# Bebra777228/PolGen-RVC

Measured on AMD Instinct MI355X. Metric: real-time-factor (audio-sec/wall-sec) per GPU, 30s@16kHz RMVPE->48kHz, higher is better.
Workload: dtype f32 (conv products as 3 fp16 MFMAs of a hi/lo split, fp32 accumulate; fp32 elsewhere)

## Files before the change

include/rvcx.h:

```cpp
#ifndef RVCX_H
#define RVCX_H
#include <stdint.h>

#ifdef __cplusplus
extern "C" {
#endif

typedef struct rvcx_ctx rvcx_ctx;

typedef struct {
  const char* name;
  const void* data;
  int32_t dtype;
  int32_t ndim;
  int64_t shape[4];
} rvcx_tensor;

typedef struct {
  int32_t inter_channels, hidden_channels, filter_channels, n_heads, n_layers, kernel_size;
  int32_t n_resblocks;
  int32_t res_kernels[4];
  int32_t res_dilations[4][3];
  int32_t n_ups;
  int32_t up_rates[6], up_kernels[6];
// ... 253 lines not shown
                   int pad_left, int Tout, int groups, int pre_lrelu, float pre_slope, int act,
                   float act_slope, const int32_t* lens_in, const int32_t* lens_out);
int rvcx_op_resblock_pair(rvcx_ctx*, const float* x, const float* w1, const float* b1, const float* w2,
                          const float* b2, float* y, int B, int C, int T, int K, int dil, float slope, int fused,
                          const int32_t* lens);
int rvcx_op_resblock3(rvcx_ctx*, const float* x, const float* w1, const float* b1, const float* w2, const float* b2,
                      float* y, int B, int C, int T, const int32_t* dils, float slope, const int32_t* lens);
int rvcx_bench_resblock_pair(rvcx_ctx*, int B, int C, int T, int K, int dil, int fused, int iters,
                             float* ms_per_launch);
int rvcx_bench_conv1d(rvcx_ctx*, int B, int Cin, int Tin, int Cout, int K, int stride, int dil, int groups,
                      int iters, float* ms_per_launch);
int rvcx_conv_override(int tile, int variant, int splitk);
int rvcx_op_convtranspose1d(rvcx_ctx*, const float* x, const float* w, const float* bias, float* y,
                            int B, int Cin, int Tin, int Cout, int K, int stride, int pad,
                            int pre_lrelu, float pre_slope);
int rvcx_op_conv2d3x3(rvcx_ctx*, const float* x, const float* w, const float* bias, const float* res,
                      float* y, int B, int Cin, int H, int W, int Cout, int act);
int rvcx_op_convblock2d(rvcx_ctx*, const float* x, const float* w1, const float* b1, const float* w2, const float* b2,
                        const float* wsc, const float* bsc, float* y, int B, int Cin, int Cout, int H, int W,
                        const int32_t* rows);
int rvcx_op_convtranspose2d(rvcx_ctx*, const float* x, const float* w, const float* bias, float* y,
                            int B, int Cin, int H, int W, int Cout, int act);
int rvcx_op_attention(rvcx_ctx*, const float* q, const float* k, const float* v, float* out, int B,
                      int H, int D, int T, float scale, const float* emb_rel_k,
                      const float* emb_rel_v, int window, const int32_t* lens);
int rvcx_op_gemm_tm(rvcx_ctx*, const float* x_cf, const float* w, const float* bias, const float* res_tm, int B, int T,
                    int Cin, int Cout, int act, int exact_fp32, float* y_tm, float* y_cf, float* y_split);
int rvcx_bench_gemm(rvcx_ctx*, int64_t rows, int Cin, int Cout, int iters, float* ms_per_launch);
int rvcx_op_layernorm_tm(rvcx_ctx*, const float* x, const float* gamma, const float* beta, float* y, float* y_split,
                         int64_t rows, int C, float eps);
// ... 35 lines not shown
```

polgen-rvc_amd/_lib.py:

```python
from __future__ import annotations

import ctypes as C
import os
import threading
import types
from typing import Optional, Sequence

import numpy as np

_HERE = os.path.dirname(os.path.abspath(__file__))
LIB_PATH = os.environ.get("RVCX_LIBRARY") or os.path.join(_HERE, "librvcx.so")


class RvcxError(RuntimeError):
    pass


class Tensor(C.Structure):
    _fields_ = [("name", C.c_char_p), ("data", C.c_void_p), ("dtype", C.c_int32),
                ("ndim", C.c_int32), ("shape", C.c_int64 * 4)]


class SynthCfg(C.Structure):
    _fields_ = [("inter_channels", C.c_int32), ("hidden_channels", C.c_int32),
# ... 98 lines not shown
    k = min(Lx, Lb)
    fin = np.sin(0.5 * np.pi * np.arange(Lx) / max(Lx - 1, 1)) ** 2
    out[:k] = y[d:d + k] * fin[:k] + b[:k] * (1.0 - fin[:k])
    return out, y[d + Lb:d + Lb + Lx].copy(), d, scores, mags


_lib = None

SYMBOLS = [
    "rvcx_create", "rvcx_destroy", "rvcx_last_error", "rvcx_version", "rvcx_load_hubert",
    "rvcx_load_rmvpe", "rvcx_index_exhaustive", "rvcx_load_crepe", "rvcx_crepe_frames", "rvcx_crepe_predict", "rvcx_op_crepe_decode", "rvcx_get_f0_crepe_x", "rvcx_load_fcpe", "rvcx_fcpe_f0", "rvcx_fcpe_frames", "rvcx_get_f0_fcpe_x", "rvcx_op_fcpe_post", "rvcx_load_synth", "rvcx_unload_synth", "rvcx_load_index", "rvcx_load_index_ivf",
    "rvcx_weights_regions", "rvcx_weights_adopt", "rvcx_weights_clone", "rvcx_rmvpe_f0", "rvcx_rmvpe_frames", "rvcx_rmvpe_mel", "rvcx_synth_infer_taps", "rvcx_hubert_features",
    "rvcx_hubert_frames", "rvcx_synth_infer", "rvcx_synth_infer_window", "rvcx_synth_dec_rf", "rvcx_synth_upp", "rvcx_index_blend",
    "rvcx_out_len", "rvcx_convert_batch", "rvcx_convert_batch_f64", "rvcx_micro_batch", "rvcx_bucket_length", "rvcx_last_micro_batches", "rvcx_last_cuts", "rvcx_noise_len",
    "rvcx_get_f0", "rvcx_get_f0_x", "rvcx_vc", "rvcx_vc_frames", "rvcx_last_timing",
    "rvcx_flop_counter", "rvcx_fp32_reruns", "rvcx_mem_info", "rvcx_conv_profile", "rvcx_conv_profile_csv", "rvcx_stream", "rvcx_op_conv1d", "rvcx_op_resblock_pair", "rvcx_bench_resblock_pair", "rvcx_bench_conv1d", "rvcx_conv_override", "rvcx_op_convtranspose1d",
    "rvcx_op_conv2d3x3", "rvcx_op_convblock2d", "rvcx_op_convtranspose2d", "rvcx_op_attention", "rvcx_op_layernorm_c",
    "rvcx_op_bigru", "rvcx_op_highpass", "rvcx_highpass_exact", "rvcx_convert_batch_ex", "rvcx_get_f0_x_ex", "rvcx_fp32_layers", "rvcx_fp32_pinned",
    "rvcx_gru_fallbacks", "rvcx_gru_publish_probe", "rvcx_debug_inject", "rvcx_f0_file_track", "rvcx_op_gemm_tm", "rvcx_op_layernorm_tm",
    "rvcx_resample_len", "rvcx_resample_f64", "rvcx_resample_f64_kind", "rvcx_bench_gemm", "rvcx_device_info",
    "rvcx_convert_submit", "rvcx_convert_wait", "rvcx_convert_poll", "rvcx_convert_inflight", "rvcx_ticket_lead_ms",
    "rvcx_synth_infer_head", "rvcx_op_sola", "rvcx_stream_open", "rvcx_stream_step", "rvcx_stream_reset", "rvcx_stream_close",
    "rvcx_stream_out_len", "rvcx_stream_noise_len", "rvcx_stream_frames",
    "rvcx_stream_open_io", "rvcx_stream_in_len", "rvcx_stream_delays", "rvcx_stream_resample_delay", "rvcx_stream_last_taps",
    "rvcx_stream_set", "rvcx_op_stream_resample",
    "rvcx_stream_open_fx", "rvcx_stream_out_channels", "rvcx_stream_set_fx", "rvcx_stream_last_fx_ms", "rvcx_op_stream_fx",
    "rvcx_fx_reverb_host",
    "rvcx_fx_chain", "rvcx_op_fx_highpass", "rvcx_op_fx_compressor", "rvcx_op_fx_gate", "rvcx_op_fx_reverb", "rvcx_op_fx_shelf",
    "rvcx_op_fx_chorus", "rvcx_op_fx_mix", "rvcx_fx_chunk", "rvcx_fx_last_passes", "rvcx_fx_cte", "rvcx_fx_delay",
    "rvcx_fx_coeffs", "rvcx_fx_highpass_host", "rvcx_fx_biquad_host", "rvcx_fx_follower_host", "rvcx_fx_compressor_host",
    "rvcx_fx_gate_host", "rvcx_fx_comb_host", "rvcx_fx_allpass_host", "rvcx_fx_chorus_host", "rvcx_fx_mix_host",
# ... 568 lines not shown
        return ms.value, flops / (ms.value * 1e-3) / 1e12

    def convtranspose1d(self, x, w, bias=None, stride=1, pad=0, pre_lrelu=None):
        x, w = f32(x), f32(w)
        B, Cin, Tin = x.shape
        _, Cout, K = w.shape
        Tout = (Tin - 1) * stride - 2 * pad + K
        y = np.empty((B, Cout, Tout), np.float32)
        bias = None if bias is None else f32(bias)
        self._ck(lib().rvcx_op_convtranspose1d(self._h, _p(x), _p(w), _p(bias), _p(y), B, Cin, Tin, Cout, K,
                                               stride, pad, 0 if pre_lrelu is None else 1,
                                               C.c_float(0.0 if pre_lrelu is None else pre_lrelu)),
                 "op_convtranspose1d")
        return y

    def conv2d3x3(self, x, w, bias=None, res=None, act=0):
        x, w = f32(x), f32(w)
        B, Cin, H, W = x.shape
        Cout = w.shape[0]
        y = np.empty((B, Cout, H, W), np.float32)
        bias = None if bias is None else f32(bias)
        res = None if res is None else f32(res)
        self._ck(lib().rvcx_op_conv2d3x3(self._h, _p(x), _p(w), _p(bias), _p(res), _p(y), B, Cin, H, W, Cout,
                                         act), "op_conv2d3x3")
        return y

    def convblock2d(self, x, w1, b1, w2, b2, wsc=None, bsc=None, rows=None):
        x, w1, w2 = f32(x), f32(w1), f32(w2)
        B, Cin, H, W = x.shape
        Cout = w1.shape[0]
# ... 771 lines not shown
            if kd[i] == 500003:
                return "resblock3 (whole k=3 ResBlock: three fused steps, persistent)"
            if kd[i] >= 500000:
                return f"resblock_pair<C={kd[i] - 500000},N1={bn[i]}> (c1 -> c2 -> +x fused)"
            if kd[i] >= 400000:
                c = kd[i] - 400000
                return f"conv_h3<{bm[i]},{bn[i]},{'linear' if c == 1 else 'stride2' if c == 2 else 'halo%d' % c}>"
            if kd[i] == 300001:
                return "conv_cout1 (vector FMA, Cout=1)"
            if kd[i] == 300003:
                return "conv_ws<64,320> (weight-stationary tile: a stage = one 16-channel chunk x all taps; K segments + finish)"
            if kd[i] == 300004:
                return "conv3_thin (3x3, C=16/32: streaming MFMA, B operand from global, DPP-shifted taps)"
            if kd[i] == 300002:
                return "convt_thin (ConvTranspose1d k4 s2, streaming MFMA + fused noise conv)"
            if kd[i] >= 300000:
                return "conv_cin1 (vector FMA, Cin=1)"
            if kd[i] >= 200000:
                return f"conv_fast_sb<{bm[i]},{bn[i]},stride2>"
            if kd[i] >= 100000:
                return f"conv_fast_sb<{bm[i]},{bn[i]},linear>"
            return f"conv_fast_sb<{bm[i]},{bn[i]},halo{kd[i] // 10}>"
        self._tile_names = [name(i) for i in range(N)]
        return [dict(tile=name(i), launches=int(la[i]), flops=float(fl[i]), ms=float(ms[i]))
                for i in range(N) if la[i] > 0]

    def conv_profile_csv(self) -> str:
        txt = (lib().rvcx_conv_profile_csv(self._h) or b"").decode()
        names = getattr(self, "_tile_names", None)
        if not names:
# ... 47 lines not shown
```

polgen-rvc_amd/csrc/api_ops.hip:

```cpp
#include "api_internal.h"
#include "h3_device.h"

using namespace rvcx;
using namespace rvcx::api;

static void to_host(Ctx& c, float* h, const float* d, size_t n) {
  RVCX_HIP(hipMemcpyAsync(h, d, n * sizeof(float), hipMemcpyDeviceToHost, c.stream));
  RVCX_HIP(hipStreamSynchronize(c.stream));
}
#define TEMP_REGION(C) WeightRegion tmp_region_; RegionScope tmp_scope_(*(C), tmp_region_)

extern "C" {

int rvcx_op_conv1d(rvcx_ctx* ctx, const float* x, const float* w, const float* bias, const float* res,
                   float* y, int B, int Cin, int Tin, int Cout, int K, int stride, int dil,
                   int pad_left, int Tout, int groups, int pre_lrelu, float pre_slope, int act,
                   float act_slope, const int32_t* lens_in, const int32_t* lens_out) {
  API_BEGIN(ctx)
  TEMP_REGION(C);
  size_t nx = (size_t)B * Cin * Tin, ny = (size_t)B * Cout * Tout;
  C->arena.reserve((nx + 2 * ny) * 4 + (64 << 20));
  C->arena.reset();
  ConvW L = make_conv(*C, w, bias, Cout, Cin / groups, K, groups, true);
  float* dx = to_dev(*C, x, nx);
// ... 297 lines not shown
  C->arena.reset();
  ConvT1dW L = make_convT1d(*C, w, bias, Cin, Cout, K, stride, pad);
  float* dx = to_dev(*C, x, nx);
  float* dy = C->arena.alloc<float>(ny);
  ConvArgs a = convT1d_args(L, dx, dy, B, Tin, Tout);
  if (pre_lrelu) {
    a.pre_act = ACT_LRELU;
    a.pre_slope = pre_slope;
  }
  C->conv(a);
  to_host(*C, y, dy, ny);
  C->arena.reset();
  API_END
}

static std::vector<float> pad_rows(const float* x, size_t planes, int H, int W) {
  const int Wp = W + 2;
  std::vector<float> o(planes * H * Wp, 0.f);
  for (size_t p = 0; p < planes; ++p)
    for (int h = 0; h < H; ++h)
      std::memcpy(&o[(p * H + h) * Wp + 1], &x[(p * H + h) * W], (size_t)W * 4);
  return o;
}
static void unpad_rows(const std::vector<float>& xp, float* y, size_t planes, int H, int W) {
  const int Wp = W + 2;
  for (size_t p = 0; p < planes; ++p)
    for (int h = 0; h < H; ++h)
      std::memcpy(&y[(p * H + h) * W], &xp[(p * H + h) * Wp + 1], (size_t)W * 4);
}

// ... 574 lines not shown
```

polgen-rvc_amd/csrc/conv.h:

```cpp
#pragma once
#include "common.h"

namespace rvcx {

enum Act { ACT_NONE = 0, ACT_LRELU = 1, ACT_RELU = 2, ACT_GELU = 3, ACT_TANH = 4, ACT_SIGMOID = 5 };
enum OutMode { OUT_NORMAL = 0, OUT_SHUF1D = 1, OUT_SHUF2D = 2, OUT_TRANSPOSED = 3 };
enum Acc2 { ACC2_NONE = 0, ACC2_SET = 1, ACC2_ADD = 2, ACC2_ADD_DIV = 3 };

struct ConvArgs {
  const float* x = nullptr;
  const float* w = nullptr;
  const void* w_h3 = nullptr;
  const void* x_split = nullptr;
  void* y_split = nullptr;
  const float* bias = nullptr;
  const float* res = nullptr;
  float* y = nullptr;
  float* y2 = nullptr;
  const int* lens_in = nullptr;
  const int* lens_out = nullptr;
  int B = 1;
  int Cin_g = 0, Cin_gp = 0, Cout_g = 0, Cout_gp = 0, groups = 1;
  int Tin = 0;
  int Nout = 0;
// ... 106 lines not shown
  double ms[kMaxTiles] = {0};
  int bm[kMaxTiles] = {0}, bn[kMaxTiles] = {0}, halo[kMaxTiles] = {0};
};
void conv_profile_begin();
void conv_profile_end(ConvProfile* out);
const char* conv_profile_csv();
void conv_init();
void launch_conv(ConvArgs a, hipStream_t stream);
int launch_conv_fast(ConvArgs& a, hipStream_t stream);
void conv_fast_describe(ConvProfile* p);
int launch_conv_h3(ConvArgs& a, int halo, int off_min, hipStream_t stream);
bool convt_thin_ok(const ConvArgs& a);
void launch_convt_thin(const ConvArgs& a, hipStream_t stream);
void convt_thin_init();
constexpr int kConvtThinSlot = 61;
bool conv3_thin_ok(const ConvArgs& a);
void launch_conv3_thin(const ConvArgs& a, hipStream_t stream);
constexpr int kConv3ThinSlot = 59;
bool conv_deep_ok(const ConvArgs& a);
void launch_conv_deep(const ConvArgs& a, hipStream_t stream);
constexpr int kConvDeepSlot = 63;
bool conv_h3_enabled();
bool conv_h3_configured();
bool conv_h3_split_ok(const ConvArgs& a);
void launch_splitk_finish(const ConvArgs& a, hipStream_t stream);
void conv_h3_describe(ConvProfile* p);
struct ConvOverride { int tile = -1, variant = -1, splitk = -1; };
extern ConvOverride g_conv_override;
void conv_fast_init();
double conv_flops(const ConvArgs& a);
// ... 16 lines not shown
```

polgen-rvc_amd/csrc/conv_fast.hip:

```cpp
#include <cmath>
#include <cstdlib>

#include "conv.h"
#include "conv_device.h"

#ifdef RVCX_ABLATION
#define RVCX_DBG(a, bit) ((a).dbg & (bit))
#else
#define RVCX_DBG(a, bit) 0
#endif

namespace rvcx {

struct BufRsrc {
#if defined(__HIP_DEVICE_COMPILE__)
  __amdgpu_buffer_rsrc_t r;
#endif
};
constexpr int kBufOob = 0x7ffffff0;
__device__ __forceinline__ BufRsrc make_rsrc(const float* base, int bytes) {
  BufRsrc b;
#if defined(__HIP_DEVICE_COMPILE__)
  b.r = __builtin_amdgcn_make_buffer_rsrc(const_cast<float*>(base), 0, bytes, 0x00020000);
#endif
// ... 431 lines not shown
  }
  if (const char* e = getenv("RVCX_STAGGER")) g_stagger_scale = (float)atof(e);
  if (const char* e = getenv("RVCX_CONV_TILE")) g_conv_override.tile = atoi(e);
}

void conv_fast_describe(ConvProfile* p) {
  p->bm[7] = 16;
  p->bn[7] = 256;
  p->halo[7] = 300000;
  p->bm[60] = 1;
  p->bn[60] = 1024;
  p->halo[60] = 300001;
  p->bm[kConvtThinSlot] = 128;
  p->bn[kConvtThinSlot] = 32;
  p->halo[kConvtThinSlot] = 300002;
  p->bm[kConv3ThinSlot] = 32;
  p->bn[kConv3ThinSlot] = 30;
  p->halo[kConv3ThinSlot] = 300004;
  p->bm[kConvDeepSlot] = 64;
  p->bn[kConvDeepSlot] = 320;
  p->halo[kConvDeepSlot] = 300003;
  for (int t = 0; t < kNumFast; ++t) {
    const int s = 8 + t;
    p->bm[s] = kFast[t].bm;
    p->bn[s] = kFast[t].bn;
    p->halo[s] = kFast[t].cic == 32 ? 100000 : (kFast[t].halo < 0 ? 200000 : kFast[t].halo * 10);
  }
}

void launch_splitk_finish(const ConvArgs& a, hipStream_t stream) {
// ... 127 lines not shown
```

polgen-rvc_amd/csrc/conv_h3.hip:

```cpp
#include <algorithm>
#include <cmath>
#include <cstdlib>

#include "conv.h"
#include "conv_device.h"
#include "h3_device.h"

#ifdef RVCX_ABLATION
#define H3_DBG(a, bit) ((a).dbg & (bit))
#else
#define H3_DBG(a, bit) 0
#endif

namespace rvcx {

template <int BM, int BN, int WR, int WC, int KKT, int HALO, int STRIDE, bool LIN, bool XS = false>
__global__ __launch_bounds__(256, ((LIN && BM * BN >= 8192) || BN >= 512) ? 2 : 3) void conv_h3_kernel(const ConvArgs a) {
  constexpr int WM = BM / (32 * WR), WN = BN / (32 * WC);
  constexpr int WROW = LIN ? BN : BN * STRIDE + HALO;
  constexpr int NBTILE = LIN ? KKT : 1;
  constexpr int A_ELEMS = KKT * 2 * 2 * BM;
  constexpr int NA = (A_ELEMS + 255) / 256;
  constexpr int B_TASKS = NBTILE * 2 * WROW;
  constexpr int NBT = (B_TASKS + 255) / 256;
// ... 366 lines not shown
    *s_out = S;
  };
  int best = -1, S = 1;
  select(1, 0, &best, &S);
  static const int tile2_mask = getenv("RVCX_TILE2_MASK") ? atoi(getenv("RVCX_TILE2_MASK")) : 255;
  const int cls = (a.out_mode != OUT_NORMAL) ? 8 : (lin ? 2 : (halo > 64 ? 1 : 4));
  int cls2 = cls;
  if (a.x_split || a.y_split) cls2 |= 16;
  const bool tile_for_batch = (tile2_mask & cls) && (!(cls2 & 16) || (tile2_mask & 16));
  if (best >= 0 && a.B > 1 && tile_for_batch) {
    int b2 = -1, s2 = 1;
    select(a.B, S, &b2, &s2);
    if (b2 >= 0 && s2 == S) best = b2;
  }
  if (best < 0) return -1;
  const H3Cfg& F = kH3[best];
  a.off_min = off_min;
  a.wrow = halo;
  a.splitk = S;
  {
    static int dbg = -1;
    if (dbg < 0) dbg = getenv("RVCX_CONV_DBG") ? atoi(getenv("RVCX_CONV_DBG")) : 0;
    a.dbg = dbg;
  }
  dim3 grid(cdiv(a.Nout, F.bn), cdiv(a.Cout_gp, F.bm), a.B * a.groups * S);
  {
    static const bool log = getenv("RVCX_CONV_LOG") != nullptr;
    if (log)
      fprintf(stderr, "h3 tile %d (%dx%d halo %d) S %d grid %u %u %u B %d Cin %d Cout %d k %d Nout %d xs %d ys %d\n", best,
              F.bm, F.bn, F.halo, S, grid.x, grid.y, grid.z, a.B, a.Cin_g, a.Cout_g, a.ksize, a.Nout, a.x_split != nullptr,
// ... 10 lines not shown
```

polgen-rvc_amd/csrc/ctx.h:

```cpp
#pragma once
#include <memory>

#include "common.h"
#include "conv.h"
#include "gemm.h"

namespace rvcx {

struct SynthModel;
struct RmvpeModel;
struct FcpeModel;
struct CrepeModel;
struct HubertModel;
struct IndexData;

class WeightRegion {
 public:
  static constexpr size_t kChunkBytes = (size_t)32 << 20;
  static constexpr int kMaxFlags = 4096;
  static constexpr size_t kHeaderBytes = kMaxFlags;
  WeightRegion() {
    flags_.reset(new uint8_t[kMaxFlags]);
    std::memset(flags_.get(), 0, kMaxFlags);
  }
// ... 43 lines not shown
    int best = 0;
    for (int i = 0; i < nflags_; ++i)
      if (w[i] > best) {
        best = w[i];
        *index = i;
      }
    if (best) RVCX_HIP(hipMemset(ovf_words_, 0, kMaxFlags * sizeof(int)));
    return best;
  }
  void clear_overflow() {
    if (ovf_words_) RVCX_HIP(hipMemset(ovf_words_, 0, kMaxFlags * sizeof(int)));
  }
  void drop_flag(int index) {
    flags_[index] = 0;
    ++dropped_;
    pinned_.push_back(index);
    if (!chunks_.empty()) RVCX_HIP(hipMemcpy(chunks_[0].base, flags_.get(), kMaxFlags, hipMemcpyHostToDevice));
  }
  int dropped() const { return dropped_; }
  void describe_flag(const uint8_t* flag, const std::string& what) {
    const size_t i = (size_t)(flag - flags_.get());
    if (desc_.size() <= i) desc_.resize(i + 1);
    desc_[i] = what;
  }
  std::string pinned_text(const std::string& region) const {
    std::string t;
    for (int i : pinned_)
      t += region + ": layer " + std::to_string(i) + " of " + std::to_string(nflags_) + " (" +
           ((size_t)i < desc_.size() && !desc_[i].empty() ? desc_[i] : std::string("?")) + ")\n";
    return t;
  }
  void seal() {
    if (chunks_.empty()) reserve(256);
    RVCX_HIP(hipMemcpy(chunks_[0].base, flags_.get(), kMaxFlags, hipMemcpyHostToDevice));
  }
  void adopt() {
    if (chunks_.empty()) return;
    RVCX_HIP(hipMemcpy(flags_.get(), chunks_[0].base, kMaxFlags, hipMemcpyDeviceToHost));
  }
  int n_chunks() const { return (int)chunks_.size(); }
  void* chunk_base(int i) const { return chunks_[i].base; }
  size_t chunk_used(int i) const { return chunks_[i].off; }
  size_t used() const {
    size_t t = 0;
    for (auto& c : chunks_) t += c.off;
    return t;
  }
  uint64_t layout_hash() const { return hash_; }

 private:
  struct Chunk {
    void* base;
    size_t cap, off;
  };
  void new_chunk(size_t bytes) {
    Chunk c{nullptr, bytes, 0};
    RVCX_HIP(hipMalloc(&c.base, bytes));
    chunks_.push_back(c);
  }
  void mix(uint64_t v) {
    for (int i = 0; i < 8; ++i) {
      hash_ ^= (v >> (8 * i)) & 0xff;
      hash_ *= 1099511628211ull;
    }
  }
  std::vector<Chunk> chunks_;
  std::unique_ptr<uint8_t[]> flags_;
  int* ovf_words_ = nullptr;
  int nflags_ = 0, dropped_ = 0;
  std::vector<int> pinned_;
  std::vector<std::string> desc_;
  uint64_t hash_ = 1469598103934665603ull;
};

class WeightSlab {
 public:
  float* upload(const std::vector<float>& h) { return cur().upload(h); }
  float* upload(const float* h, size_t n) { return cur().upload(h, n); }
  uint8_t* new_flag(bool v) { return cur().new_flag(v); }
  WeightRegion& cur() {
    if (!cur_) fail("internal: weight upload outside a RegionScope");
    return *cur_;
  }
  WeightRegion* cur_ = nullptr;
// ... 190 lines not shown
```

polgen-rvc_amd/csrc/models.h:

```cpp
#pragma once
#include <functional>

#include "../../include/rvcx.h"
#include "ctx.h"
#include "layers.h"

namespace rvcx {

struct SynthModel {
  std::shared_ptr<WeightRegion> region = std::make_shared<WeightRegion>();
  rvcx_synth_cfg cfg{};
  int upp = 1;
  int dec_rf_frames = 0;
  ConvW emb_phone;
  const float* emb_pitch = nullptr;
  struct EncLayer {
    ConvW qkv, o, ffn1, ffn2;
    AttFlag att;
    const float *rel_k = nullptr, *rel_v = nullptr;
    const float *g1 = nullptr, *b1 = nullptr, *g2 = nullptr, *b2 = nullptr;
  };
  std::vector<EncLayer> enc;
  ConvW proj;
  struct Flow {
// ... 1 lines not shown
  };
  Flow flows[4];
  ConvW conv_pre, cond, conv_post;
  const float* lin_wb = nullptr;
  struct Stage {
    ConvT1dW up;
    ConvW noise;
    int noise_stride = 1, noise_pad = 0;
    ConvW noise_dense;
    int noise_dense_cin = 0;
    int ch = 0;
    ConvW c1[4][3], c2[4][3];
  };
  std::vector<Stage> stages;
  const float* emb_g = nullptr;
};

std::unique_ptr<SynthModel> synth_load(Ctx& c, const rvcx_synth_cfg& cfg, const TensorTable& t);

struct SynthIO {
  int B = 1, T = 0;
  const int* lens_host = nullptr;
  const float* phone_ct = nullptr;
  const int* pitch = nullptr;
  const float* pitchf = nullptr;
  const int* sid_host = nullptr;
  const float* z_noise = nullptr;
  const float* src_noise = nullptr;
  float* out = nullptr;
  int dec_skip = 0;
// ... 149 lines not shown
```

polgen-rvc_amd/csrc/synth.hip:

```cpp
#include <algorithm>
#include <cmath>
#include <cstdlib>

#include "models.h"
#include "ops.h"

namespace rvcx {

std::vector<float> wn_weight(const TensorTable& t, const std::string& p, int dim) {
  if (t.has(p + ".weight")) return t.f32(p + ".weight");
  std::string gn = p + ".parametrizations.weight.original0", vn = p + ".parametrizations.weight.original1";
  if (!t.has(gn)) {
    gn = p + ".weight_g";
    vn = p + ".weight_v";
  }
  std::vector<float> g = t.f32(gn), v = t.f32(vn);
  const auto shp = t.shape(vn);
  RVCX_CHECK(shp.size() == 3, "weight-norm tensor must be 3-D: " + p);
  const int64_t d0 = shp[0], d1 = shp[1], d2 = shp[2];
  std::vector<float> w(v.size());
  if (dim == 0) {
    RVCX_CHECK((int64_t)g.size() == d0, "weight_g shape: " + p);
    for (int64_t a = 0; a < d0; ++a) {
      double ss = 0.0;
// ... 108 lines not shown
          }
      S.noise_dense = make_conv(c, w2.data(), b1.data(), co, sp, 3, 1, true);
      S.noise_dense_cin = sp;
    }
    S.ch = co;
    for (int j = 0; j < cfg.n_resblocks; ++j)
      for (int m = 0; m < 3; ++m) {
        const std::string rp = "dec.resblocks." + std::to_string(i * cfg.n_resblocks + j);
        S.c1[j][m] = load_conv(c, t, rp + ".convs1." + std::to_string(m), true, true, true);
        S.c2[j][m] = load_conv(c, t, rp + ".convs2." + std::to_string(m), true, true, true);
      }
    M->stages.push_back(S);
    ch = co;
  }
  M->emb_g = c.slab.upload(t.f32("emb_g.weight"));
  {
    double rf = 3.0, rate = 1.0;
    for (int i = 0; i < cfg.n_ups; ++i) {
      rf += ((cfg.up_kernels[i] - 1) / cfg.up_rates[i] + 1) / rate;
      rate *= cfg.up_rates[i];
      int res = 0;
      for (int j = 0; j < cfg.n_resblocks; ++j) {
        int r = 0;
        for (int d = 0; d < 3; ++d) r += (cfg.res_kernels[j] - 1) / 2 * (cfg.res_dilations[j][d] + 1);
        res = std::max(res, r);
      }
      rf += res / rate;
    }
    rf += 3.0 / rate;
    M->dec_rf_frames = (int)std::ceil(rf) + 2;
// ... 21 lines not shown
namespace {

struct Timer3 {
  Ctx& c;
  hipEvent_t* e;
  Timer3(Ctx& cc, hipEvent_t* ev) : c(cc), e(ev) {}
  void mark(int i) {
    if (e) RVCX_HIP(hipEventRecord(e[i], c.stream));
  }
};

int* upload_ints(Ctx& c, const std::vector<int>& v) {
  int* d = c.arena.alloc<int>(v.size());
  RVCX_HIP(hipMemcpyAsync(d, v.data(), v.size() * sizeof(int), hipMemcpyHostToDevice, c.stream));
  return d;
}

}

void synth_forward(Ctx& c, const SynthModel& m, const SynthIO& io, hipEvent_t* stage_ev) {
  const auto& cf = m.cfg;
  const int B = io.B, T = io.T, hid = cf.hidden_channels, inter = cf.inter_channels, filt = cf.filter_channels;
  const int heads = cf.n_heads, kc = hid / heads, half = inter / 2, gin = cf.gin_channels;
  hipStream_t s = c.stream;
  Arena& A = c.arena;
  Timer3 tm(c, stage_ev);
  tm.mark(0);
  const int head = io.skip_head, Tk = T - head;
  RVCX_CHECK(head >= 0 && Tk > 0, "synth: skip_head outside [0, T)");
  if (head > 0) {
// ... 116 lines not shown
  {
    launch_mask(x, B, hid, T, lens, s);
    ConvArgs a = conv1d_args(m.proj, x, stats, B, T, T);
    a.lens_out = lens;
    c.conv(a);
  }
  tm.mark(1);

  float* z = A.alloc<float>((size_t)B * inter * T);
  float* z2 = A.alloc<float>((size_t)B * inter * T);
  launch_sample_z(stats, io.z_noise, z, B, inter, T, lens, s);
  if (head > 0) {
    launch_copy_strided(z + head, z2, B * inter, Tk, T, Tk, s);
    std::swap(z, z2);
  }
  float* g = A.alloc<float>((size_t)B * gin);
  for (int b = 0; b < B; ++b)
    RVCX_HIP(hipMemcpyAsync(g + (size_t)b * gin, m.emb_g + (size_t)sidv[b] * gin, gin * sizeof(float),
                            hipMemcpyDeviceToDevice, s));
  {
    float* h = att;
    float* xin = qkv;
    float* acts = tmp;
    float* rs = hbuf;
    RVCX_CHECK(filt >= 2 * hid, "buffer reuse assumes filter_channels >= 2*hidden");
    float* wout = A.alloc<float>((size_t)B * hid * T);
    float* mbuf = A.alloc<float>((size_t)B * half * T);
    float* gc = A.alloc<float>((size_t)B * 6 * hid);
    for (int f = 3; f >= 0; --f) {
      const auto& F = m.flows[f];
      launch_flip_channels(z, z2, B, inter, Tk, s);
      std::swap(z, z2);
      ConvArgs a = conv1d_args(F.pre, z, h, B, Tk, Tk);
      a.x_bs = (long)inter * Tk;
      a.lens_out = lens;
      c.conv(a);
      a = conv1d_args(F.cond, g, gc, B, 1, 1);
      c.conv(a);
      for (int i = 0; i < 3; ++i) {
        a = conv1d_args(F.in_l[i], h, xin, B, Tk, Tk, 1, 1, (F.in_l[i].k - 1) / 2);
        a.lens_in = lens;
        a.lens_out = lens;
        c.conv(a);
        launch_wn_gate(xin, gc, i * 2 * hid, 6 * hid, acts, B, hid, Tk, s);
        a = conv1d_args(F.rs_l[i], acts, rs, B, Tk, Tk);
        a.lens_out = lens;
        c.conv(a);
        launch_wn_res_skip(h, wout, rs, B, hid, Tk, i == 2, i == 0, lens, s);
      }
      a = conv1d_args(F.post, wout, mbuf, B, Tk, Tk);
      a.lens_out = lens;
      c.conv(a);
      launch_coupling_sub(z, mbuf, B, half, Tk, lens, s);
// ... 15 lines not shown
  for (int b0 = 0; b0 < B; b0 += dec_batch) {
    const int db = std::min(dec_batch, B - b0);
    A.reset(dec_mark);
    const bool own = io.lens_host != nullptr && (db == 1 || equal_lens);
    const int Tfull = own ? io.lens_host[b0] - head : Tk;
    RVCX_CHECK(Tfull > 0 && Tfull <= Tk, "synth: item length outside (0, T]");
    const int skip = (io.dec_skip > 0 && (own || !lens) && Tfull - 2 * io.dec_skip > 2 * m.dec_rf_frames) ? io.dec_skip : 0;
    const int Td = Tfull - 2 * skip;
    float* cur = A.alloc<float>((size_t)db * C0 * Td);
    {
      ConvArgs a = conv1d_args(m.conv_pre, z + (size_t)b0 * inter * Tk + skip, cur, db, Td, Td, 1, 1, 3);
      a.x_bs = (long)inter * Tk;
      a.x_cs = Tk;
      a.lens_in = (lens && !own) ? lens + b0 : nullptr;
      c.conv(a);
      float* gcond = A.alloc<float>((size_t)db * C0);
      a = conv1d_args(m.cond, g + (size_t)b0 * gin, gcond, db, 1, 1);
      c.conv(a);
      launch_add_channel_bias(cur, gcond, db, C0, Td, s);
    }
    long Tin = Td, Tin_c = Tk, off = skip;
    for (size_t i = 0; i < m.stages.size(); ++i) {
      const auto& S = m.stages[i];
      const long Tout = Tin * cf.up_rates[i], Tout_c = Tin_c * cf.up_rates[i];
      off *= cf.up_rates[i];
      const size_t n = (size_t)db * S.ch * Tout;
      float* xs = A.alloc<float>(n);
      const size_t stage_mark = A.mark();
      float* xu = A.alloc<float>(n);
      const int nk = cf.n_resblocks;
      float* xcb[4];
      float* xtb[4];
      for (int j = 0; j < nk; ++j) {
        xcb[j] = A.alloc<float>(n);
// ... 168 lines not shown
```

Before: 1242.

## Add wide ConvTranspose1d MFMA kernel and cache speaker-conditioning projections

Adds a dedicated split-fp16 MFMA kernel for the stride-10/12 ConvTranspose1d upsampling layers (k = 2·stride). It converts each input tile to hi/lo halves once in LDS and streams weights from global, with double-buffered A fragments. It also caches the per-speaker cond and flow-cond 1x1 conv outputs in a small device table keyed by speaker id and invalidated by a weights epoch, which removes the repeated tiny convs and per-item memcpys on each call. The cache reuses precomputed weight-derived results across calls but still depends on sid. The new kernel adds a code path whose precision and coverage differ from the generic h3 path.

```diff
diff --git a/include/rvcx.h b/include/rvcx.h
--- a/include/rvcx.h
+++ b/include/rvcx.h
@@ -291,6 +291,9 @@
 int rvcx_op_convtranspose1d(rvcx_ctx*, const float* x, const float* w, const float* bias, float* y,
                             int B, int Cin, int Tin, int Cout, int K, int stride, int pad,
                             int pre_lrelu, float pre_slope);
+int rvcx_op_convt1d(rvcx_ctx*, const float* x, const float* w, const float* bias, const float* res, float* y, int B, int Cin,
+                    int Tin, int Cout, int K, int stride, int pad, int pre_lrelu, float pre_slope, const int32_t* lens,
+                    int skip, const float* har, const float* nz_w, const float* nz_b, int nz_k, int nz_stride, int nz_pad);
 int rvcx_op_conv2d3x3(rvcx_ctx*, const float* x, const float* w, const float* bias, const float* res,
                       float* y, int B, int Cin, int H, int W, int Cout, int act);
 int rvcx_op_convblock2d(rvcx_ctx*, const float* x, const float* w1, const float* b1, const float* w2, const float* b2,
diff --git a/polgen-rvc_amd/_lib.py b/polgen-rvc_amd/_lib.py
--- a/polgen-rvc_amd/_lib.py
+++ b/polgen-rvc_amd/_lib.py
@@ -136,7 +136,7 @@
     "rvcx_hubert_frames", "rvcx_synth_infer", "rvcx_synth_infer_window", "rvcx_synth_dec_rf", "rvcx_synth_upp", "rvcx_index_blend",
     "rvcx_out_len", "rvcx_convert_batch", "rvcx_convert_batch_f64", "rvcx_micro_batch", "rvcx_bucket_length", "rvcx_last_micro_batches", "rvcx_last_cuts", "rvcx_noise_len",
     "rvcx_get_f0", "rvcx_get_f0_x", "rvcx_vc", "rvcx_vc_frames", "rvcx_last_timing",
-    "rvcx_flop_counter", "rvcx_fp32_reruns", "rvcx_mem_info", "rvcx_conv_profile", "rvcx_conv_profile_csv", "rvcx_stream", "rvcx_op_conv1d", "rvcx_op_resblock_pair", "rvcx_bench_resblock_pair", "rvcx_bench_conv1d", "rvcx_conv_override", "rvcx_op_convtranspose1d",
+    "rvcx_flop_counter", "rvcx_fp32_reruns", "rvcx_mem_info", "rvcx_conv_profile", "rvcx_conv_profile_csv", "rvcx_stream", "rvcx_op_conv1d", "rvcx_op_resblock_pair", "rvcx_bench_resblock_pair", "rvcx_bench_conv1d", "rvcx_conv_override", "rvcx_op_convtranspose1d", "rvcx_op_convt1d",
     "rvcx_op_conv2d3x3", "rvcx_op_convblock2d", "rvcx_op_convtranspose2d", "rvcx_op_attention", "rvcx_op_layernorm_c",
     "rvcx_op_bigru", "rvcx_op_highpass", "rvcx_highpass_exact", "rvcx_convert_batch_ex", "rvcx_get_f0_x_ex", "rvcx_fp32_layers", "rvcx_fp32_pinned",
     "rvcx_gru_fallbacks", "rvcx_gru_publish_probe", "rvcx_debug_inject", "rvcx_f0_file_track", "rvcx_op_gemm_tm", "rvcx_op_layernorm_tm",
@@ -735,6 +735,25 @@
                  "op_convtranspose1d")
         return y
 
+    def convt1d(self, x, w, bias=None, stride=10, pre_lrelu=None, lens=None, skip=0, res=None, har=None, nz_w=None,
+                nz_b=None, nz_stride=1, nz_pad=0):
+        x, w = f32(x), f32(w)
+        B, Cin, Tin = x.shape
+        _, Cout, K = w.shape
+        y = np.empty((B, Cout, (Tin - 2 * skip) * stride), np.float32)
+        bias = None if bias is None else f32(bias)
+        res = None if res is None else f32(res)
+        har = None if har is None else f32(har)
+        nz_w = None if nz_w is None else f32(nz_w)
+        nz_b = None if nz_b is None else f32(nz_b)
+        li = i32(lens)
+        self._ck(lib().rvcx_op_convt1d(self._h, _p(x), _p(w), _p(bias), _p(res), _p(y), B, Cin, Tin, Cout, K, stride,
+                                       (K - stride) // 2, 0 if pre_lrelu is None else 1,
+                                       C.c_float(0.0 if pre_lrelu is None else pre_lrelu), _p(li, C.c_int32), skip,
+                                       _p(har), _p(nz_w), _p(nz_b), 0 if nz_w is None else nz_w.shape[-1], nz_stride,
+                                       nz_pad), "op_convt1d")
+        return y
+
     def conv2d3x3(self, x, w, bias=None, res=None, act=0):
         x, w = f32(x), f32(w)
         B, Cin, H, W = x.shape
@@ -1536,6 +1555,8 @@
                 return "conv3_thin (3x3, C=16/32: streaming MFMA, B operand from global, DPP-shifted taps)"
             if kd[i] == 300002:
                 return "convt_thin (ConvTranspose1d k4 s2, streaming MFMA + fused noise conv)"
+            if kd[i] == 300005:
+                return "convt_wide (ConvTranspose1d k = 2 stride, stride 10 / 12: input tile split once, weights from global)"
             if kd[i] >= 300000:
                 return "conv_cin1 (vector FMA, Cin=1)"
             if kd[i] >= 200000:
diff --git a/polgen-rvc_amd/csrc/api_ops.hip b/polgen-rvc_amd/csrc/api_ops.hip
--- a/polgen-rvc_amd/csrc/api_ops.hip
+++ b/polgen-rvc_amd/csrc/api_ops.hip
@@ -335,6 +335,61 @@
   API_END
 }
 
+int rvcx_op_convt1d(rvcx_ctx* ctx, const float* x, const float* w, const float* bias, const float* res, float* y, int B, int Cin,
+                    int Tin, int Cout, int K, int stride, int pad, int pre_lrelu, float pre_slope, const int32_t* lens,
+                    int skip, const float* har, const float* nz_w, const float* nz_b, int nz_k, int nz_stride, int nz_pad) {
+  API_BEGIN(ctx)
+  TEMP_REGION(C);
+  if (K != 2 * stride || 2 * pad != K - stride || skip < 0 || Tin - 2 * skip < 1) fail("op_convt1d: k = 2 stride, pad = stride / 2, 0 <= 2 skip < Tin");
+  if (har && (res || !nz_w || nz_k < 1 || nz_stride < 1)) fail("op_convt1d: har excludes res and needs the noise conv's weights");
+  const int Td = Tin - 2 * skip;
+  const long Tout = (long)Td * stride, Tfull = (long)Tin * stride;
+  const size_t nx = (size_t)B * Cin * Tin, ny = (size_t)B * Cout * Tout, nr = (size_t)B * Cout * Tfull;
+  const size_t nh = har ? (size_t)B * Tfull * nz_stride : 0;
+  C->arena.reserve((nx + ny + nr + nh) * 4 + (64 << 20));
+  C->arena.reset();
+  ConvT1dW L = make_convT1d(*C, w, bias, Cin, Cout, K, stride, pad);
+  float* dx = to_dev(*C, x, nx);
+  float* dy = C->arena.alloc<float>(ny);
+  RVCX_HIP(hipMemsetAsync(dy, 0xff, ny * sizeof(float), C->stream));
+  ConvArgs a = convT1d_args(L, dx + skip, dy, B, Td, (int)Tout);
+  a.x_bs = (long)Cin * Tin;
+  a.x_cs = Tin;
+  if (pre_lrelu) {
+    a.pre_act = ACT_LRELU;
+    a.pre_slope = pre_slope;
+  }
+  std::vector<int32_t> lo, ln;
+  if (lens) {
+    for (int b = 0; b < B; ++b) {
+      if (lens[b] < 0 || lens[b] > Td) fail("op_convt1d: lens outside [0, Tin - 2 skip]");
+      lo.push_back(lens[b] * stride);
+      ln.push_back(lens[b] * stride * nz_stride);
+    }
+    a.lens_in = to_dev(*C, lens, B);
+    a.lens_out = to_dev(*C, lo.data(), B);
+  }
+  if (res) {
+    conv_set_res(a, to_dev(*C, res, nr) + (long)skip * stride, Cout, (int)Tfull);
+  } else if (har) {
+    ConvW N = make_conv(*C, nz_w, nz_b, Cout, 1, nz_k, 1, false);
+    a.nz_har = to_dev(*C, har, nh) + (long)skip * stride * nz_stride;
+    a.nz_bs = Tfull * nz_stride;
+    a.nz_w = N.w;
+    a.nz_wstride = N.cin_gp * N.cout_gp;
+    a.nz_b = N.bias;
+    a.nz_k = nz_k;
+    a.nz_stride = nz_stride;
+    a.nz_pad = nz_pad;
+    a.nz_len = (int)(Tout * nz_stride);
+    a.nz_lens = lens ? to_dev(*C, ln.data(), B) : nullptr;
+  }
+  C->conv(a);
+  to_host(*C, y, dy, ny);
+  C->arena.reset();
+  API_END
+}
+
 static std::vector<float> pad_rows(const float* x, size_t planes, int H, int W) {
   const int Wp = W + 2;
   std::vector<float> o(planes * H * Wp, 0.f);
diff --git a/polgen-rvc_amd/csrc/conv.h b/polgen-rvc_amd/csrc/conv.h
--- a/polgen-rvc_amd/csrc/conv.h
+++ b/polgen-rvc_amd/csrc/conv.h
@@ -144,6 +144,9 @@
 void launch_convt_thin(const ConvArgs& a, hipStream_t stream);
 void convt_thin_init();
 constexpr int kConvtThinSlot = 61;
+bool convt_wide_ok(const ConvArgs& a);
+void launch_convt_wide(const ConvArgs& a, hipStream_t stream);
+constexpr int kConvtWideSlot = 65;
 bool conv3_thin_ok(const ConvArgs& a);
 void launch_conv3_thin(const ConvArgs& a, hipStream_t stream);
 constexpr int kConv3ThinSlot = 59;
diff --git a/polgen-rvc_amd/csrc/conv_fast.hip b/polgen-rvc_amd/csrc/conv_fast.hip
--- a/polgen-rvc_amd/csrc/conv_fast.hip
+++ b/polgen-rvc_amd/csrc/conv_fast.hip
@@ -469,6 +469,9 @@
   p->bm[kConvtThinSlot] = 128;
   p->bn[kConvtThinSlot] = 32;
   p->halo[kConvtThinSlot] = 300002;
+  p->bm[kConvtWideSlot] = 256;
+  p->bn[kConvtWideSlot] = 64;
+  p->halo[kConvtWideSlot] = 300005;
   p->bm[kConv3ThinSlot] = 32;
   p->bn[kConv3ThinSlot] = 30;
   p->halo[kConv3ThinSlot] = 300004;
diff --git a/polgen-rvc_amd/csrc/conv_h3.hip b/polgen-rvc_amd/csrc/conv_h3.hip
--- a/polgen-rvc_amd/csrc/conv_h3.hip
+++ b/polgen-rvc_amd/csrc/conv_h3.hip
@@ -404,6 +404,10 @@
     if (b2 >= 0 && s2 == S) best = b2;
   }
   if (best < 0) return -1;
+  if (S == 1 && convt_wide_ok(a)) {
+    launch_convt_wide(a, stream);
+    return kConvtWideSlot;
+  }
   const H3Cfg& F = kH3[best];
   a.off_min = off_min;
   a.wrow = halo;
diff --git a/polgen-rvc_amd/csrc/convt_wide.hip b/polgen-rvc_amd/csrc/convt_wide.hip
--- /dev/null
+++ b/polgen-rvc_amd/csrc/convt_wide.hip
@@ -0,0 +1,171 @@
+#include <cstdlib>
+#include <mutex>
+
+#include "conv.h"
+#include "conv_device.h"
+#include "h3_device.h"
+
+namespace rvcx {
+
+namespace {
+
+constexpr int kWideBN = 64, kWideRow = kWideBN + 1;
+constexpr int kWideBM = 256;
+constexpr int kWideSeg = 16;
+constexpr size_t kWideLds = (size_t)kWideSeg * 4 * kWideRow * 16;
+
+__global__ __launch_bounds__(256, 2) void convt_wide_kernel(const ConvArgs a) {
+  extern __shared__ uint4 Bs[];
+  const int tid = threadIdx.x, lane = tid & 63, wave = tid >> 6;
+  const int i = lane & 31, h = lane >> 5;
+  const int b = blockIdx.z;
+  const int n0 = blockIdx.x * kWideBN;
+  const int co_w = blockIdx.y * kWideBM + wave * 64;
+  const int len_in = a.lens_in ? a.lens_in[b] : a.Tin;
+  const int len_out = a.lens_out ? a.lens_out[b] : 0x7fffffff;
+  const int nchunk = a.Cin_gp / 16;
+  const int xrow = a.x_cs * 4;
+  const H3Rsrc xr = h3_rsrc(a.x + (long)b * a.x_bs, a.Cin_g * a.x_cs * 4);
+  const H3Rsrc wr = h3_rsrc(a.w_h3, 2 * nchunk * 4 * a.Cout_gp * 16);
+  const int pre_act = a.pre_act;
+  const float pre_slope = a.pre_slope;
+  const bool dead = n0 * a.sh_s - a.sh_pad >= len_out;
+  const bool rows = co_w < a.Cout_gp;
+
+  f32x16 acc[2][2];
+#pragma unroll
+  for (int m = 0; m < 2; ++m)
+#pragma unroll
+    for (int n = 0; n < 2; ++n)
+#pragma unroll
+      for (int r = 0; r < 16; ++r) acc[m][n][r] = 0.f;
+
+  const int slab = 4 * a.Cout_gp * 16;
+  int a_off[2];
+#pragma unroll
+  for (int m = 0; m < 2; ++m) a_off[m] = co_w + m * 32 < a.Cout_gp ? (h * a.Cout_gp + co_w + m * 32 + i) * 16 : kH3Oob;
+  const int op_bytes = 2 * a.Cout_gp * 16;
+  auto load_a = [&](uint4* f, int c, int kk) {
+    const int base = (kk * nchunk + c) * slab;
+#pragma unroll
+    for (int m = 0; m < 2; ++m) {
+      const bool ok = a_off[m] != kH3Oob && c < nchunk;
+      f[2 * m + 0] = h3_load4(wr, ok ? base + a_off[m] : kH3Oob);
+      f[2 * m + 1] = h3_load4(wr, ok ? base + op_bytes + a_off[m] : kH3Oob);
+    }
+  };
+  uint4 a0[4], a1[4];
+  if (rows && !dead) load_a(a0, 0, 0);
+
+  bool ovf = false;
+  for (int c0 = 0; c0 < nchunk && !dead; c0 += kWideSeg) {
+    const int nc = min(kWideSeg, nchunk - c0);
+    if (c0 > 0) __syncthreads();
+    const int ntask = nc * 2 * kWideRow;
+#pragma unroll 2
+    for (int t = tid; t < ntask; t += 256) {
+      const int ch8 = t / kWideRow, p = t - ch8 * kWideRow;
+      const int pos = n0 - 1 + p;
+      const bool ok = pos >= 0 && pos < len_in;
+      const int off = ((c0 * 2 + ch8) * 8) * xrow + pos * 4;
+      float v[8];
+#pragma unroll
+      for (int q = 0; q < 8; ++q) v[q] = h3_load1(xr, ok ? off + q * xrow : kH3Oob);
+      half8 hi, lo;
+#pragma unroll
+      for (int q = 0; q < 8; ++q) {
+        float x = v[q];
+        if (pre_act == ACT_LRELU) x = x > 0.f ? x : x * pre_slope;
+        ovf |= !(fabsf(x) < kH3ActLimit);
+        const _Float16 xh = (_Float16)x;
+        hi[q] = xh;
+        lo[q] = (_Float16)((x - (float)xh) * kH3Scale);
+      }
+      const int e = ((ch8 >> 1) * 4 + (ch8 & 1)) * kWideRow + p;
+      Bs[e] = __builtin_bit_cast(uint4, hi);
+      Bs[e + 2 * kWideRow] = __builtin_bit_cast(uint4, lo);
+    }
+    __syncthreads();
+    if (!rows) continue;
+    auto step = [&](const uint4* ac, int cl, int kk) {
+      const uint4* Bt = Bs + cl * 4 * kWideRow + i + kk;
+      half8 af[3][2], bf[2][2];
+#pragma unroll
+      for (int m = 0; m < 2; ++m) {
+        af[0][m] = __builtin_bit_cast(half8, ac[2 * m + 0]);
+        af[2][m] = __builtin_bit_cast(half8, ac[2 * m + 1]);
+        af[1][m] = af[0][m] * (_Float16)(1.f / kH3Scale);
+      }
+#pragma unroll
+      for (int op = 0; op < 2; ++op)
+#pragma unroll
+        for (int n = 0; n < 2; ++n) bf[op][n] = __builtin_bit_cast(half8, Bt[(op * 2 + h) * kWideRow + n * 32]);
+#pragma unroll
+      for (int m = 0; m < 2; ++m)
+#pragma unroll
+        for (int n = 0; n < 2; ++n) {
+          acc[m][n] = h3_mfma(af[0][m], bf[0][n], acc[m][n]);
+          acc[m][n] = h3_mfma(af[1][m], bf[1][n], acc[m][n]);
+          acc[m][n] = h3_mfma(af[2][m], bf[0][n], acc[m][n]);
+        }
+    };
+    for (int cl = 0; cl < nc; ++cl) {
+      load_a(a1, c0 + cl, 1);
+      __builtin_amdgcn_sched_barrier(0);
+      step(a0, cl, 0);
+      __builtin_amdgcn_sched_barrier(0);
+      load_a(a0, c0 + cl + 1, 0);
+      __builtin_amdgcn_sched_barrier(0);
+      step(a1, cl, 1);
+      __builtin_amdgcn_sched_barrier(0);
+    }
+  }
+  if (ovf) report_h3_overflow(a.ovf, a.ovf_layer, a.seq);
+  if (!rows) return;
+  constexpr float inv = 1.f / kH3Scale;
+  auto finish = [&](f32x16 t, int m, int n) {
+#pragma unroll
+    for (int r = 0; r < 16; ++r) t[r] *= inv;
+    store_tile_shuf1d(a, b, co_w + m * 32 + 4 * h, n0 + n * 32 + i, t, len_out);
+  };
+  finish(acc[0][0], 0, 0);
+  finish(acc[0][1], 0, 1);
+  finish(acc[1][0], 1, 0);
+  finish(acc[1][1], 1, 1);
+}
+
+}
+
+bool convt_wide_ok(const ConvArgs& a) {
+  static const bool on = !getenv("RVCX_UP_WIDE") || atoi(getenv("RVCX_UP_WIDE")) != 0;
+  if (!on || g_conv_override.tile >= 0 || g_conv_override.splitk > 1) return false;
+  if (!a.w_h3 || a.out_mode != OUT_SHUF1D || !(a.sh_s == 10 || a.sh_s == 12) || a.ksize != 2 || a.kw != 2 || a.pad != 1 ||
+      a.stride != 1 || a.dil != 1 || a.groups != 1)
+    return false;
+  if (a.Cin_g % 16 != 0 || a.Cin_gp != a.Cin_g || a.Cout_gp % 32 != 0) return false;
+  if (a.x_split || a.y_split || a.acc2_mode != ACC2_NONE || a.act != ACT_NONE || a.zero_wp != 0) return false;
+  if (!(a.pre_act == ACT_NONE || a.pre_act == ACT_LRELU)) return false;
+  if ((long)a.Cin_g * a.x_cs * 4 >= kH3Oob || (long)2 * a.Cin_gp * a.Cout_gp * 4 >= kH3Oob) return false;
+  if (cdiv(a.Cout_gp, kWideBM) > 65535 || a.B > 65535) return false;
+  return conv_h3_enabled();
+}
+
+void launch_convt_wide(const ConvArgs& a, hipStream_t stream) {
+  {
+    static std::mutex mu;
+    static uint64_t done = 0;
+    int dev = 0;
+    RVCX_HIP(hipGetDevice(&dev));
+    std::lock_guard<std::mutex> g(mu);
+    if (!((done >> (dev & 63)) & 1)) {
+      RVCX_HIP(hipFuncSetAttribute(reinterpret_cast<const void*>(convt_wide_kernel), hipFuncAttributeMaxDynamicSharedMemorySize,
+                                   (int)kWideLds));
+      done |= 1ull << (dev & 63);
+    }
+  }
+  dim3 grid(cdiv(a.Nout, kWideBN), cdiv(a.Cout_gp, kWideBM), a.B);
+  hipLaunchKernelGGL(convt_wide_kernel, grid, dim3(256), kWideLds, stream, a);
+  RVCX_HIP(hipGetLastError());
+}
+
+}
diff --git a/polgen-rvc_amd/csrc/ctx.h b/polgen-rvc_amd/csrc/ctx.h
--- a/polgen-rvc_amd/csrc/ctx.h
+++ b/polgen-rvc_amd/csrc/ctx.h
@@ -81,6 +81,7 @@
   void drop_flag(int index) {
     flags_[index] = 0;
     ++dropped_;
+    ++epoch_;
     pinned_.push_back(index);
     if (!chunks_.empty()) RVCX_HIP(hipMemcpy(chunks_[0].base, flags_.get(), kMaxFlags, hipMemcpyHostToDevice));
   }
@@ -104,7 +105,9 @@
   void adopt() {
     if (chunks_.empty()) return;
     RVCX_HIP(hipMemcpy(flags_.get(), chunks_[0].base, kMaxFlags, hipMemcpyDeviceToHost));
-  }
+    ++epoch_;
+  }
+  uint64_t epoch() const { return epoch_; }
   int n_chunks() const { return (int)chunks_.size(); }
   void* chunk_base(int i) const { return chunks_[i].base; }
   size_t chunk_used(int i) const { return chunks_[i].off; }
@@ -135,6 +138,7 @@
   std::unique_ptr<uint8_t[]> flags_;
   int* ovf_words_ = nullptr;
   int nflags_ = 0, dropped_ = 0;
+  uint64_t epoch_ = 0;
   std::vector<int> pinned_;
   std::vector<std::string> desc_;
   uint64_t hash_ = 1469598103934665603ull;
diff --git a/polgen-rvc_amd/csrc/models.h b/polgen-rvc_amd/csrc/models.h
--- a/polgen-rvc_amd/csrc/models.h
+++ b/polgen-rvc_amd/csrc/models.h
@@ -39,6 +39,15 @@
   };
   std::vector<Stage> stages;
   const float* emb_g = nullptr;
+  struct CondCache {
+    static constexpr int kSlots = 4;
+    float* buf = nullptr;
+    int per = 0;
+    int sid[kSlots] = {-1, -1, -1, -1};
+    uint64_t epoch = 0;
+    int next = 0;
+  };
+  mutable CondCache cond_cache;
 };
 
 std::unique_ptr<SynthModel> synth_load(Ctx& c, const rvcx_synth_cfg& cfg, const TensorTable& t);
diff --git a/polgen-rvc_amd/csrc/synth.hip b/polgen-rvc_amd/csrc/synth.hip
--- a/polgen-rvc_amd/csrc/synth.hip
+++ b/polgen-rvc_amd/csrc/synth.hip
@@ -146,6 +146,8 @@
     ch = co;
   }
   M->emb_g = c.slab.upload(t.f32("emb_g.weight"));
+  M->cond_cache.per = cfg.up_initial_channel + 4 * 6 * cfg.hidden_channels;
+  M->cond_cache.buf = static_cast<float*>(c.slab.cur().reserve((size_t)SynthModel::CondCache::kSlots * M->cond_cache.per * sizeof(float)));
   {
     double rf = 3.0, rate = 1.0;
     for (int i = 0; i < cfg.n_ups; ++i) {
@@ -197,6 +199,74 @@
   int* d = c.arena.alloc<int>(v.size());
   RVCX_HIP(hipMemcpyAsync(d, v.data(), v.size() * sizeof(int), hipMemcpyHostToDevice, c.stream));
   return d;
+}
+
+__global__ __launch_bounds__(256) void cond_gather_kernel(const float* table, const int* slot, int per, int C0, int h6, int B,
+                                                          float* gcond, float* gflow) {
+  const int b = blockIdx.x;
+  const float* src = table + (long)slot[b] * per;
+  for (int j = threadIdx.x; j < per; j += 256) {
+    const float v = src[j];
+    if (j < C0) {
+      gcond[(long)b * C0 + j] = v;
+    } else {
+      const int r = j - C0, f = r / h6, q = r - f * h6;
+      gflow[((long)f * B + b) * h6 + q] = v;
+    }
+  }
+}
+
+bool cond_from_table(Ctx& c, const SynthModel& m, const std::vector<int>& sidv, const float** gcond, const float* gflow[4]) {
+  static const bool on = !getenv("RVCX_COND_CACHE") || atoi(getenv("RVCX_COND_CACHE")) != 0;
+  SynthModel::CondCache& cc = m.cond_cache;
+  if (!on || !cc.buf || g_force_fp32) return false;
+  constexpr int kSlots = SynthModel::CondCache::kSlots;
+  if (cc.epoch != m.region->epoch()) {
+    for (int& v : cc.sid) v = -1;
+    cc.epoch = m.region->epoch();
+  }
+  std::vector<int> need;
+  for (int v : sidv)
+    if (std::find(need.begin(), need.end(), v) == need.end()) need.push_back(v);
+  if ((int)need.size() > kSlots) return false;
+  const int C0 = m.cfg.up_initial_channel, h6 = 6 * m.cfg.hidden_channels, gin = m.cfg.gin_channels, B = (int)sidv.size();
+  auto slot_of = [&](int sid) {
+    for (int k = 0; k < kSlots; ++k)
+      if (cc.sid[k] == sid) return k;
+    return -1;
+  };
+  for (int sid : need) {
+    if (slot_of(sid) >= 0) continue;
+    int k = cc.next;
+    while (cc.sid[k] >= 0 && std::find(need.begin(), need.end(), cc.sid[k]) != need.end()) k = (k + 1) % kSlots;
+    cc.next = (k + 1) % kSlots;
+    cc.sid[k] = -1;
+    float* dst = cc.buf + (size_t)k * cc.per;
+    const float* g = m.emb_g + (size_t)sid * gin;
+    ConvArgs a = conv1d_args(m.cond, g, dst, 1, 1, 1);
+    c.conv(a);
+    for (int f = 3; f >= 0; --f) {
+      a = conv1d_args(m.flows[f].cond, g, dst + C0 + (size_t)f * h6, 1, 1, 1);
+      c.conv(a);
+    }
+    cc.sid[k] = sid;
+  }
+  if (B == 1) {
+    const float* row = cc.buf + (size_t)slot_of(sidv[0]) * cc.per;
+    *gcond = row;
+    for (int f = 0; f < 4; ++f) gflow[f] = row + C0 + (size_t)f * h6;
+    return true;
+  }
+  std::vector<int> slots(B);
+  for (int b = 0; b < B; ++b) slots[b] = slot_of(sidv[b]);
+  const int* dslots = upload_ints(c, slots);
+  float* gc = c.arena.alloc<float>((size_t)B * C0);
+  float* gf = c.arena.alloc<float>((size_t)4 * B * h6);
+  hipLaunchKernelGGL(cond_gather_kernel, dim3(B), dim3(256), 0, c.stream, cc.buf, dslots, cc.per, C0, h6, B, gc, gf);
+  RVCX_HIP(hipGetLastError());
+  *gcond = gc;
+  for (int f = 0; f < 4; ++f) gflow[f] = gf + (size_t)f * B * h6;
+  return true;
 }
 
 }
@@ -343,10 +413,16 @@
     launch_copy_strided(z + head, z2, B * inter, Tk, T, Tk, s);
     std::swap(z, z2);
   }
-  float* g = A.alloc<float>((size_t)B * gin);
-  for (int b = 0; b < B; ++b)
-    RVCX_HIP(hipMemcpyAsync(g + (size_t)b * gin, m.emb_g + (size_t)sidv[b] * gin, gin * sizeof(float),
-                            hipMemcpyDeviceToDevice, s));
+  const float* gcond_tab = nullptr;
+  const float* gflow_tab[4] = {nullptr, nullptr, nullptr, nullptr};
+  const bool cond_tab = cond_from_table(c, m, sidv, &gcond_tab, gflow_tab);
+  float* g = nullptr;
+  if (!cond_tab) {
+    g = A.alloc<float>((size_t)B * gin);
+    for (int b = 0; b < B; ++b)
+      RVCX_HIP(hipMemcpyAsync(g + (size_t)b * gin, m.emb_g + (size_t)sidv[b] * gin, gin * sizeof(float),
+                              hipMemcpyDeviceToDevice, s));
+  }
   {
     float* h = att;
     float* xin = qkv;
@@ -355,7 +431,7 @@
     RVCX_CHECK(filt >= 2 * hid, "buffer reuse assumes filter_channels >= 2*hidden");
     float* wout = A.alloc<float>((size_t)B * hid * T);
     float* mbuf = A.alloc<float>((size_t)B * half * T);
-    float* gc = A.alloc<float>((size_t)B * 6 * hid);
+    float* gc_own = cond_tab ? nullptr : A.alloc<float>((size_t)B * 6 * hid);
     for (int f = 3; f >= 0; --f) {
       const auto& F = m.flows[f];
       launch_flip_channels(z, z2, B, inter, Tk, s);
@@ -364,8 +440,11 @@
       a.x_bs = (long)inter * Tk;
       a.lens_out = lens;
       c.conv(a);
-      a = conv1d_args(F.cond, g, gc, B, 1, 1);
-      c.conv(a);
+      const float* gc = cond_tab ? gflow_tab[f] : gc_own;
+      if (!cond_tab) {
+        a = conv1d_args(F.cond, g, gc_own, B, 1, 1);
+        c.conv(a);
+      }
       for (int i = 0; i < 3; ++i) {
         a = conv1d_args(F.in_l[i], h, xin, B, Tk, Tk, 1, 1, (F.in_l[i].k - 1) / 2);
         a.lens_in = lens;
@@ -411,10 +490,14 @@
       a.x_cs = Tk;
       a.lens_in = (lens && !own) ? lens + b0 : nullptr;
       c.conv(a);
-      float* gcond = A.alloc<float>((size_t)db * C0);
-      a = conv1d_args(m.cond, g + (size_t)b0 * gin, gcond, db, 1, 1);
-      c.conv(a);
-      launch_add_channel_bias(cur, gcond, db, C0, Td, s);
+      if (cond_tab) {
+        launch_add_channel_bias(cur, gcond_tab + (size_t)b0 * C0, db, C0, Td, s);
+      } else {
+        float* gcond = A.alloc<float>((size_t)db * C0);
+        a = conv1d_args(m.cond, g + (size_t)b0 * gin, gcond, db, 1, 1);
+        c.conv(a);
+        launch_add_channel_bias(cur, gcond, db, C0, Td, s);
+      }
     }
     long Tin = Td, Tin_c = Tk, off = skip;
     for (size_t i = 0; i < m.stages.size(); ++i) {
```

Result: no change. 1249 (median of 6 runs) (+0.6%).
